# marvinx97/cloud

Hardware: AMD Instinct MI355X
Metric: images/sec ResNet-50 via run() at 1/2/4/8 MI355X; run()→first-step latency (higher is better)
Workload: dtype bf16

## Files before the change

cloud_amd/config.py:

```python
from __future__ import annotations

import os
from dataclasses import dataclass


@dataclass(frozen=True)
class Var:
    name: str
    type: type
    default: object
    doc: str
    area: str


_VARS = [
    Var("CLOUD_AMD_JOBS_DIR", str, "./jobs", "where run() stages job directories", "launcher"),
    Var("CLOUD_AMD_HOME", str, "~/.cloud_amd", "per-user state: the job-id index (jobs/<id> -> job directory) that "
        "python -m cloud_amd.jobs uses to find a job from any directory", "launcher"),
    Var("CLOUD_AMD_STAGE_COPY", bool, False, "stage code files by copying too (default: code "
        "hard-linked, every other file copied; a running job then never sees in-place edits of its sources)", "launcher"),
    Var("CLOUD_AMD_CPU_AFFINITY", bool, True, "launcher pins each GPU rank to the cores of its GPU's NUMA node "
        "(KFD io_links + sysfs cpulist), split between the ranks on that node; 0 = leave placement to the OS",
        "launcher"),
    Var("CLOUD_AMD_NUMA_ROOT", str, "/sys/devices/system/node", "sysfs NUMA-node tree read for rank CPU placement "
# ... 46 lines not shown
    Var("CLOUD_AMD_BN_APPLY_BLOCKS", int, 0, "BatchNorm apply passes (fwd y/mask, bwd dz): total workgroups of "
        "the HBM stream; 0 = the reduction kernels' tiling", "ops"),
    Var("CLOUD_AMD_BN_APPLY_ILV", bool, True, "BatchNorm apply passes: 1 = RP-row groups dealt round-robin to "
        "the workgroups (one contiguous sweep); 0 = one contiguous row chunk per workgroup", "ops"),
    Var("CLOUD_AMD_CONV_TALL", bool, True, "<= 64-channel 3x3 convolutions (fwd, stride-1 dgrad): 256 x 64 tiles "
        "with 4 x 1 waves; 0 = 128 x 64 with 2 x 2 waves", "ops"),
    Var("CLOUD_AMD_STEM_LDS", bool, True, "space-to-depth stem convolution forward on the LDS-resident patch + filter "
        "kernel (csrc/include/ca_conv_stem.h); 0 = the implicit-GEMM row-segment loader", "ops"),
    Var("CLOUD_AMD_STEM_TALL", bool, True, "space-to-depth stem convolution on the tall 256 x 64 tiles too (0.88 -> "
        "0.72 ms per call at b1024); 0 = 128 x 64 tiles (A/B runs)", "ops"),
    Var("CLOUD_AMD_STEM_BWD_RECOMPUTE", bool, True, "ResNet stem tail backward: a statistics-only max-pool "
        "backward pass, then the BN-backward apply recomputes the pooled gradient per 2x2 block (the 112x112 "
        "gradient is never written: 3.3 GB fewer per step at b1024).  With the window loads issued ahead of "
        "any branch: 0.65 + 0.90 ms against 1.09 + 0.94 for write-then-apply, +0.8 % end to end "
        "(profiles/r4_s44/); 0 = write g and run the separate apply pass", "ops"),
    Var("CLOUD_AMD_BN_GROUPS_MAX", int, 512, "BatchNorm statistics: most groups of the first-level reduction of the "
        "per-tile partial rows (1..512; ~64 rows per group)", "ops"),
    Var("CLOUD_AMD_GEMM_LIB", str, "never", "plain bf16 GEMMs (bias / accumulate only, no fused epilogue): 'never' "
        "(default: every GEMM on the in-tree kernels, the same engine on every box and rank), 'auto' (diagnostic: "
        "times the in-tree kernel against hipBLASLt once per shape and keeps the faster), 'always' "
        "(ops/raw.py PlainGemmPolicy)", "ops"),
    Var("CLOUD_AMD_GEMM_PRW", bool, True, "forward 1x1 convolutions with N = 256, K = 64 (ResNet layer-1 conv3 "
        "and shortcut): persistent resident-weight core (csrc/include/ca_gemm_prw.h); 0 = the tiled 128 core",
        "ops"),
    Var("CLOUD_AMD_GEMM_PRWN", bool, True, "forward 1x1 convolutions N = 512 / K = 128 and N = 1024 / K = 256 with "
        "BN statistics (ResNet stage-2 / stage-3 conv3): the persistent core with the weight resident in column "
        "chunks (ca_gemm_prw.h); 0 = the tiled 128 core", "ops"),
    Var("CLOUD_AMD_SMALLK_SET", str, "", "bench/smallk_gemm.py shape set ('conv3': the conv3 expansions of "
        "stages 2-4)", "bench"),
    Var("CLOUD_AMD_EPI_PF", bool, True, "GEMM epilogues that read memory or run an activation (BN-statistics "
        "forward 1x1 convs, BERT bias/GELU/GELU'/beta dense layers): 4 staged output rows in flight per trip", "ops"),
    Var("CLOUD_AMD_ATTN_FUSED_BWD", bool, True, "attention at S = 64 / 128: one workgroup per (batch, head) for "
        "the forward and a single fused backward kernel; 0 keeps the 64-query-block kernels", "ops"),
    Var("CLOUD_AMD_CONV_HALO_WGRAD", bool, True, "the weight gradient of the same 3x3 / 64-channel / width-56 "
        "convolutions on the LDS-resident kernel (ca_conv_halo.h conv3x3_halo_wgrad: 64 x 576 partial in registers, "
        "one fp32 slab per workgroup); 0 = implicit GEMM (A/B)", "ops"),
    Var("CLOUD_AMD_LN_BWD16", bool, False, "LayerNorm backward on 16-wave blocks, one row per wave, the block's "
        "partials summed by a fixed LDS tree (measured 2.8 % slower on BERT beside the weight-gradient side stream; "
        "default: 4-wave blocks walking four rows per wave)", "ops"),
    Var("CLOUD_AMD_GEMM_256X96", bool, True, "forward GEMMs whose 256 x 96 grid fills whole rounds while the 128 x "
        "128 grid leaves a partial one (BERT QKV, M = 8192, N = 2304) run on 256 x 96 tiles; 0 = off (A/B)", "ops"),
    Var("CLOUD_AMD_BN_FIN_RPG", int, 512, "BatchNorm statistics finalize: partial rows per group block (64-512)", "ops"),
    Var("CLOUD_AMD_BN_FIN_MERGED", bool, True, "BatchNorm statistics from many partial rows: group reduction and "
        "per-channel finalize in ONE launch (last block per 64 channels finalizes, agent-scope ticket); 0 = two "
        "launches (A/B runs)", "ops"),
    Var("CLOUD_AMD_CONV_HALO", int, 1, "3x3 / stride-1 / 64-channel convolutions at width 56 (ResNet-50 "
        "stage 1) forward and input gradient on the LDS-resident kernel (ca_conv_halo.h: input patch and all 9 taps "
        "in LDS, persistent grid); 0 = implicit-GEMM tiles, 2 = halo kernel without the software-pipelined "
        "fragment reads (A/B runs)", "ops"),
    Var("CLOUD_AMD_CONV_PATCH", bool, True, "3x3 / stride-1 / pad-1 convolutions with a 64-multiple gathered channel "
        "count, more than 64 output columns and W <= 28 (ResNet-50 stages 2-4), forward and input gradient, on the "
        "patch-fed core (ca_conv_patch.h: the tile's input rows go to LDS once per 64-channel chunk, not once per "
        "tap); 0 = tap-gathered implicit GEMM (A/B runs)", "ops"),
    Var("CLOUD_AMD_CONV_EPI_PF", bool, True, "implicit-GEMM forward convolutions with the BN-statistics epilogue: "
        "read 2 staged output rows from LDS before storing", "ops"),
    Var("CLOUD_AMD_SHAPE_LOG", str, None, "profiling: append one JSON line per GEMM/convolution launch (kind, M, N, "
        "K, minimum HBM bytes) to this file, for scripts/gemm_roofline.py", "ops"),
    Var("CLOUD_AMD_BN_FOLD", bool, True, "ResNet block backward: the bn3 / bn1 backward apply runs in the operand "
        "fetch of the 1x1 input-gradient GEMM that consumes it (ca_gemm_xa.h) instead of a separate pass", "ops"),
    Var("CLOUD_AMD_BN_FOLD_FWD", bool, True, "ResNet block forward: bn2's apply runs in conv3's operand fetch and "
        "bn3's (+ residual) in the next block's conv1 (ca_gemm_xa.h); the applied tensors are written once, by "
        "those GEMMs", "ops"),
    Var("CLOUD_AMD_BN_FOLD_MAX_N", int, 256, "BN fold sites kept: only GEMMs with K >= 2N and N <= this "
        "(ResNet-50 default: bn3 -> conv3 dgrad and bn3 -> next conv1 at stages 1-3, the stage-3 ones on the two-deep "
        "128 x 256 transform-A tiles, CLOUD_AMD_XA_N256=3: +0.6 / +1.0 % on two boxes, docs/performance.md round 6; "
        "4096 = every stage); the short-K sites (bn2 -> conv3, bn1 -> conv1 dgrad) measured slower than the separate "
        "pass, and stage 4 (N 512) +0.3 % below stages 1-3 only", "ops"),
    Var("CLOUD_AMD_BN_FOLD_WGRAD", bool, True, "bn3 -> conv3 fold at 64 input channels (ResNet stage 1): conv3's weight "
        "gradient runs in the same kernel as its input gradient (ca_gemm_xa.h mfma_gemm_xa_dw), so the BN-backward "
        "output dz3 is never written", "ops"),
    Var("CLOUD_AMD_BN_FOLD_DS", bool, False, "ResNet projection blocks, stages 2-4: the shortcut BN's backward apply "
        "runs in the operand fetch of the sparse strided shortcut input-gradient GEMM (ca_gemm_xa_bwd_strided); A/B",
        "ops"),
    Var("CLOUD_AMD_DS_SPARSE_DGRAD", bool, True, "ResNet projection blocks with a strided 1x1 shortcut: the "
        "shortcut's input gradient is written for its one non-empty output-parity class only, and conv1's input "
        "gradient accumulates into it reading the other pixels as zeros -- no zero-fill of 3/4 of dx and no read "
        "of those zeros", "ops"),
    Var("CLOUD_AMD_BN_FOLD_WGRAD_DS", bool, True, "stage-1 projection shortcut: its BN backward (gated by the block "
        "output's ReLU mask), the shortcut conv's input gradient and its weight gradient in one pass", "ops"),
    Var("CLOUD_AMD_BN_FOLD_WGRAD2", bool, False, "the same one-pass input + weight gradient for stage 2's conv3 "
        "(K = 512 -> N = 128, 8-wave workgroups holding the 512 x 128 dW block)", "ops"),
    Var("CLOUD_AMD_BN_FOLD_WGRAD1", bool, False, "the same one-pass input + weight gradient for stage 1's conv1 with "
        "bn1's backward apply (K = 64 -> N = 256: dz1 never written, four output chunks per tile)", "ops"),
    Var("CLOUD_AMD_XA_N256", int, 3, "transform-A GEMMs (BN folded into a 1x1 conv) with N a multiple of 256: "
        "1 = 128 x 256 tiles on 16-wave workgroups (each A tile transformed once), "
        "3 (and any other value) = 16 waves with two K tiles' operands in flight (coefficients staged in LDS; K <= 2048), "
        "0 = 128 x 128 tiles.  Only the fold sites CLOUD_AMD_BN_FOLD_MAX_N admits reach them (ResNet-50 stage 3 "
        "at the default; measured in docs/performance.md, round 6)", "ops"),
    Var("CLOUD_AMD_XA_WAVES", int, 8,"128 x 128 transform-A GEMMs (BN folded into the 1x1 convs): 8-wave "
        "workgroups (<= 128 registers, two per CU) or 4", "ops"),
    Var("CLOUD_AMD_XA_WAVES_N64", bool, True, "the 128 x 64 transform-A GEMMs (stage 1) on 8-wave workgroups too "
        "(with CLOUD_AMD_XA_WAVES=8)", "ops"),
    Var("CLOUD_AMD_XA_DW_WAVES", int, 4, "stage-1 conv3 fused input+weight gradient: 4-wave workgroups (two per "
        "CU) or 8 (one per CU); 8 selects the one-step form", "ops"),
    Var("CLOUD_AMD_XA_DW_DEPTH", int, 1, "stage-1 fused input+weight gradient (K 256 -> N 64): 0 = one-step form; "
        "1, 2, 4 = deep form (weights resident in LDS, epilogue operands ahead of the next tile's) with that many "
        "source steps in flight per workgroup (1: two workgroups per CU, 2 and 4: one)", "ops"),
    Var("CLOUD_AMD_BN_FOLD_ALL", bool, False, "fold every BN site regardless of CLOUD_AMD_BN_FOLD_MAX_N (tests, A/B)",
        "ops"),
    Var("CLOUD_AMD_MAX_STEPS_IN_FLIGHT", int, 2, "training loops (benches, Keras fit) let the host enqueue at most this "
        "many steps ahead of the GPU (runtime.step_pacer); bounds the memory in flight so the caching allocator "
        "stops requesting segments after warmup; 0 = unbounded", "runtime"),
    Var("CLOUD_AMD_RUN_AHEAD_MS", float, 25.0, "the step pacer deepens its bound (up to 4 steps) so the queued steps "
        "cover at least this much GPU time, measured on the first steps: short steps (BERT-base 8.7 ms -> 3) "
        "absorb host hiccups, long ones keep CLOUD_AMD_MAX_STEPS_IN_FLIGHT; 0 = fixed depth", "runtime"),
    Var("CLOUD_AMD_GC_FREEZE", bool, True, "training loops (benches, Keras fit) call runtime.gc_control.freeze() after "
# ... 140 lines not shown
```

cloud_amd/ops/raw.py:

```python
from __future__ import annotations

import json
import os

import torch

from . import _ext

NT, NN, TN = 0, 1, 2

_SHAPE_LOG = os.environ.get("CLOUD_AMD_SHAPE_LOG") or None


def _log(kind, M, N, K, nbytes, **kw):
    if _SHAPE_LOG is None:
        return
    with open(_SHAPE_LOG, "a") as f:
        f.write(json.dumps(dict(kind=kind, M=int(M), N=int(N), K=int(K), bytes=int(nbytes), **kw)) + "\n")


def _nb(*ts):
    if _SHAPE_LOG is None:
        return 0
    return sum(t.numel() * t.element_size() for t in ts if t is not None)
# ... 99 lines not shown
        if is_gemm_conv(w, stride, padding):
            part = torch.empty(((N * H * W + 127) // 128, 2, Cin), dtype=torch.float32, device=dy.device)
            if beta_stride > 1:
                ext.dgrad_gemm(NN, dy.data_ptr(), Cout, w.data_ptr(), Cin, dx.data_ptr(), Cin, N * H * W, Cin, Cout,
                               float(beta), 0, 0, z.data_ptr(), _ext.ptr(mask), part.data_ptr(), _st(dy.device),
                               par_s=int(beta_stride), par_h=H, par_w=W)
            else:
                ext.gemm_bf16_bnstats(NN, dy.data_ptr(), Cout, w.data_ptr(), Cin, dx.data_ptr(), Cin, N * H * W, Cin,
                                      Cout, float(beta), z.data_ptr(), _ext.ptr(mask), part.data_ptr(), _st(dy.device))
            _log("dgrad1x1_bn", N * H * W, Cin, Cout, _nb(dy, w, dx, z, mask) + (_nb(dx) if beta else 0))
        else:
            rows = ext.conv_dgrad_stat_rows(N, H, W, Cin, Cout, KH, KW, stride, stride, padding, padding,
                                            float(beta))
            part = torch.empty((rows, 2, Cin), dtype=torch.float32, device=dy.device)
            ext.conv_dgrad_bnstats(dy.data_ptr(), w.data_ptr(), dx.data_ptr(), N, H, W, Cin, Cout, KH, KW, stride,
                                   stride, padding, padding, float(beta), z.data_ptr(), _ext.ptr(mask),
                                   part.data_ptr(), _st(dy.device))
            _log("dgrad%dx%ds%d_bn" % (KH, KW, stride), N * H * W, Cin, Cout * KH * KW, _nb(dy, w, dx, z, mask),
                 launches=stride * stride)
        return dx, part
    if is_gemm_conv(w, stride, padding):
        if beta_stride > 1:
            ext.dgrad_gemm(NN, dy.data_ptr(), Cout, w.data_ptr(), Cin, dx.data_ptr(), Cin, N * H * W, Cin, Cout,
                           float(beta), 0, 0, 0, 0, 0, _st(dy.device), par_s=int(beta_stride), par_h=H, par_w=W)
        else:
            ext.gemm_bf16(NN, dy.data_ptr(), Cout, w.data_ptr(), Cin, dx.data_ptr(), Cin, N * H * W, Cin, Cout, 0,
                          float(beta), _st(dy.device))
        _log("dgrad1x1", N * H * W, Cin, Cout, _nb(dy, w, dx) + (_nb(dx) // beta_stride ** 2 if beta else 0))
        return dx
    if skip_empty:
        assert beta == 0 and stride > 1, "skip_empty: strided convolutions, beta 0"
    ext.conv_dgrad(dy.data_ptr(), w.data_ptr(), dx.data_ptr(), N, H, W, Cin, Cout, KH, KW, stride, stride, padding,
                   padding, float(beta), _st(dy.device), skip_empty=int(bool(skip_empty)))
    _log("dgrad%dx%ds%d" % (KH, KW, stride), N * H * W, Cin, Cout * KH * KW, _nb(dy, w, dx), launches=stride * stride)
    return dx


def conv_wgrad(dy, x, w_shape, stride, padding, out, beta=1.0, blocks=None):
    global _WGRAD_BLOCKS, _WGRAD_BLOCKS_SMALLM
    ext = _ext.load(required=True)
    if _WGRAD_BLOCKS is None:
        from .. import config

        _WGRAD_BLOCKS = config.get("CLOUD_AMD_WGRAD_BLOCKS")
        _WGRAD_BLOCKS_SMALLM = config.get("CLOUD_AMD_WGRAD_BLOCKS_SMALLM")
    N, H, W, Cin = x.shape
    Cout, KH, KW, _ = w_shape
    OH, OW = dy.shape[1], dy.shape[2]
    kred = N * OH * OW
    ncols = KH * KW * Cin
    target = blocks or (_WGRAD_BLOCKS_SMALLM if Cout <= 128 else _WGRAD_BLOCKS)
    splits = ext.gemm_splitk_effective(kred, wgrad_splits(Cout, ncols, kred, target_blocks=target))
    if not (KH == 1 and KW == 1):
        splits = ext.conv_wgrad_splits(N, H, W, Cin, Cout, KH, KW, stride, stride, padding, padding, splits)
    ws = torch.empty(splits * Cout * ncols, dtype=torch.float32, device=x.device)
    obf = int(out.dtype == torch.bfloat16)
    if KH == 1 and KW == 1 and stride == 1 and padding == 0:
        ext.gemm_splitk(TN, dy.data_ptr(), Cout, x.data_ptr(), Cin, out.data_ptr(), obf, float(beta), Cout, Cin,
                        kred, splits, ws.data_ptr(), _st(x.device))
    else:
        ext.conv_wgrad(dy.data_ptr(), x.data_ptr(), out.data_ptr(), obf, float(beta), N, H, W, Cin, Cout, KH, KW,
                       stride, stride, padding, padding, splits, ws.data_ptr(), _st(x.device))
    _log("wgrad%dx%ds%d" % (KH, KW, stride), Cout, ncols, kred, _nb(dy, x, out) + (2 * _nb(ws) if splits > 1 else 0),
         splits=splits)
    return out


XA_BN_RELU, XA_BN_RES_RELU, XA_BN_BWD, XA_BN_RESBN_RELU = 0, 1, 2, 3


def conv1x1_dgrad_bnbwd(dy, z, mask, coef, w, side, out=None, beta=0.0, bn=None, res=None):
    ext = _ext.load(required=True)
    N, H, W, Cout = z.shape
    Cin = w.shape[3]
    M = N * H * W
    x_shape = (N, H, W, Cin)
    assert dy.shape == z.shape and side.shape == z.shape and w.shape[1:3] == (1, 1)
    assert dy.is_contiguous() and z.is_contiguous() and side.is_contiguous() and coef.numel() == 3 * Cout
    assert mask is None or mask.shape == (M, Cout // 8)
    dx = out if out is not None else torch.empty(x_shape, dtype=torch.bfloat16, device=dy.device)
    src, rmask, zp, mp, part, part2, z2p = 0, 0, 0, 0, None, None, 0
    if res is not None:
        src_t, rm_t = res
        assert src_t.shape == dx.shape and src_t.is_contiguous()
        src, rmask = src_t.data_ptr(), _ext.ptr(rm_t)
    if bn is not None:
        zb, mb = bn[0], bn[1]
        assert zb.shape == dx.shape and zb.is_contiguous() and (mb is None or mb.shape == (M, Cin // 8))
        part = torch.empty(((M + 127) // 128, 2, Cin), dtype=torch.float32, device=dy.device)
        zp, mp = zb.data_ptr(), _ext.ptr(mb)
        if len(bn) > 2 and bn[2] is not None:
            assert res is not None, "second-BN statistics need the residual-gated (res=) form"
            part2 = torch.empty_like(part)
            z2p = bn[2].data_ptr()
    cp = coef.data_ptr()
    ext.gemm_xa(NN, XA_BN_BWD, dy.data_ptr(), z.data_ptr(), _ext.ptr(mask), cp, cp + 4 * Cout, cp + 8 * Cout, 0,
                side.data_ptr(), 0, Cout, w.data_ptr(), Cin, dx.data_ptr(), Cin, M, Cin, Cout, float(beta), src, rmask,
                zp, mp, _ext.ptr(part), z2p, _ext.ptr(part2), _st(dy.device))
    _log("dgrad1x1_xa", M, Cin, Cout, _nb(dy, z, mask, side, w, dx) + (_nb(dx) if beta else 0))
    if bn is None:
        return dx
    return (dx, part, part2) if (len(bn) > 2 and bn[2] is not None) else (dx, part)


def conv1x1_strided_dgrad_bnbwd(dy, z, mask, coef, w, side, x_shape, stride):
    ext = _ext.load(required=True)
    N, Ho, Wo, Cout = z.shape
# ... 525 lines not shown
```

csrc/bindings.cpp:

```cpp
#include <atomic>
#include <mutex>
#include <hip/hip_runtime.h>
#include <pybind11/pybind11.h>
#include <pybind11/stl.h>
#include <stdint.h>

#include <stdexcept>
#include <string>
#include <vector>

namespace py = pybind11;
typedef uint16_t bf16_t;

extern "C" {
int ca_sgd_step(float*, void*, int, float*, bf16_t*, const float*, const float*, long, int, int, hipStream_t);
int ca_adam_step(float*, void*, int, float*, float*, bf16_t*, const float*, const float*, long, int, int, hipStream_t);
int ca_rmsprop_step(float*, void*, int, float*, float*, bf16_t*, const float*, const float*, long, int, hipStream_t);
int ca_sumsq(const void*, int, long, float*, hipStream_t);
int ca_scale(void*, int, long, const float*, hipStream_t);
long ca_bn_workspace_floats(long, int);
int ca_bn_fwd(const bf16_t*, const bf16_t*, bf16_t*, long, int, const float*, const float*, float, float,
              float*, float*, float*, float*, float*, float*, int, uint8_t*, hipStream_t);
int ca_bn_apply(const bf16_t*, const bf16_t*, bf16_t*, long, int, const float*, int, hipStream_t);
int ca_bn_fwd_partials(const bf16_t*, const bf16_t*, bf16_t*, long, int, const float*, int, const float*, const float*,
                       float, float, float*, float*, float*, float*, float*, int, uint8_t*, float*, hipStream_t);
int ca_bn_bwd(const bf16_t*, const bf16_t*, const uint8_t*, const bf16_t*, long, int, const float*, const float*,
              const float*, bf16_t*, bf16_t*, float*, float*, float*, float*, int, hipStream_t);
int ca_bn_bwd_partials(const bf16_t*, const bf16_t*, const uint8_t*, const bf16_t*, long, int, const float*, int,
                       const float*, const float*, const float*, bf16_t*, bf16_t*, float*, float*, float*, float*, int,
                       hipStream_t);
int ca_gemm_bf16_bnstats(int, const bf16_t*, long, const bf16_t*, long, bf16_t*, long, int, int, int, float,
                         const bf16_t*, const uint8_t*, float*, hipStream_t);
long ca_conv_dgrad_stat_tiles(int, int, int, int, int);
long ca_conv_dgrad_stat_rows(int, int, int, int, int, int, int, int, int, int, int, float);
int ca_conv_patch_shape(int, int, int, int, int, int, int, int, int, int, int, int);
long ca_conv_stat_rows(int, int, int, int, int, int, int, int, int, int, int);
int ca_conv_wgrad_splits(int, int, int, int, int, int, int, int, int, int, int, int);
int ca_bn_fwd_partials_ex(const bf16_t*, const bf16_t*, const float*, bf16_t*, long, int, const float*, int,
                          const float*, const float*, float, float, float*, float*, float*, float*, float*, int,
                          uint8_t*, float*, hipStream_t);
int ca_gemm_xa(int, int, const bf16_t*, const bf16_t*, const uint8_t*, const float*, const float*, const float*,
               const float*, bf16_t*, uint8_t*, long, const bf16_t*, long, bf16_t*, long, int, int, int, float, const bf16_t*,
               const uint8_t*, const bf16_t*, const uint8_t*, float*, const bf16_t*, float*, hipStream_t);
int ca_gemm_xa_bwd_strided(const bf16_t*, const bf16_t*, const uint8_t*, const float*, const float*, const float*,
                           bf16_t*, long, const bf16_t*, long, bf16_t*, long, int, int, int, int, int, int, int,
                           hipStream_t);
int ca_gemm_xa_dw(const bf16_t*, const bf16_t*, const uint8_t*, const float*, const float*, const float*, long,
                  const bf16_t*, long, bf16_t*, long, int, int, int, float, const bf16_t*, const uint8_t*,
                  const bf16_t*, const uint8_t*, float*, const bf16_t*, float*, const bf16_t*, long, void*, int, float,
                  float*, int, hipStream_t);
int ca_dgrad_gemm(int, const bf16_t*, long, const bf16_t*, long, bf16_t*, long, int, int, int, float, const bf16_t*,
                  const uint8_t*, const bf16_t*, const uint8_t*, float*, hipStream_t, const bf16_t*, float*, int, int,
                  int);
int ca_conv_dgrad_bnstats(const bf16_t*, const bf16_t*, bf16_t*, int, int, int, int, int, int, int, int, int, int,
                          int, float, const bf16_t*, const uint8_t*, float*, hipStream_t);
int ca_u8_normalize(const uint8_t*, bf16_t*, long, int, const float*, const float*, hipStream_t);
int ca_stem_s2d(const bf16_t*, bf16_t*, int, int, int, int, int, int, int, hipStream_t);
int ca_softmax_xent(const void*, int, const int64_t*, int, int, float, float, float*, float*, void*, hipStream_t);
int ca_softmax_xent_batch(const void*, long, int, const int64_t*, int, int, float, float, float*, float*, void*, float*,
                          float,
                          hipStream_t);
int ca_maxpool_fwd(const bf16_t*, bf16_t*, uint8_t*, int, int, int, int, int, int, int, int, int, hipStream_t);
int ca_maxpool_bwd(const bf16_t*, const uint8_t*, bf16_t*, int, int, int, int, int, int, int, int, int, hipStream_t);
int ca_gap_fwd(const bf16_t*, void*, int, int, int, int, hipStream_t);
int ca_gap_bwd(const void*, int, bf16_t*, int, int, int, hipStream_t);
int ca_gmp_fwd(const bf16_t*, bf16_t*, float*, int, int, int, hipStream_t);
int ca_gmp_bwd(const void*, int, const bf16_t*, const bf16_t*, const float*, bf16_t*, int, int, int, hipStream_t);
int ca_gemm_bf16(int, const bf16_t*, long, const bf16_t*, long, bf16_t*, long, int, int, int, float*, float,
                 hipStream_t);
int ca_gemm_set_core(int);
int ca_gemm_set_xa_n256(int);
int ca_gemm_stat_rows(int, int, int, long, long, long);
int ca_bn_relu_maxpool_s2k3(const bf16_t*, const float*, bf16_t*, uint8_t*, int, int, int, int, int, int, hipStream_t);
int ca_maxpool_bnstats_parts(int, int, int, int);
int ca_maxpool_bwd_s2k3_bnstats(const bf16_t*, const bf16_t*, const uint8_t*, const bf16_t*, bf16_t*, float*, int, int,
                                int, int, int, int, hipStream_t);
int ca_maxpool_bwd_s2k3_bnapply(const bf16_t*, const bf16_t*, const uint8_t*, const bf16_t*, const float*, bf16_t*, int,
                                int, int, int, int, int, hipStream_t);
int ca_conv_fwd_ex(const bf16_t*, const bf16_t*, bf16_t*, int, int, int, int, int, int, int, int, int, int, int,
                   const float*, int, hipStream_t);
int ca_conv_fwd(const bf16_t*, const bf16_t*, bf16_t*, int, int, int, int, int, int, int, int, int, int, int, float*,
                hipStream_t);
int ca_conv_dgrad(const bf16_t*, const bf16_t*, bf16_t*, int, int, int, int, int, int, int, int, int, int, int, float,
                  hipStream_t, int);
int ca_conv_wgrad(const bf16_t*, const bf16_t*, void*, int, float, int, int, int, int, int, int, int, int, int, int,
                  int, int, float*, hipStream_t);
int ca_splitk_reduce(const float*, int, long, void*, int, float, hipStream_t);
int ca_grad_finalize_multi(const uint64_t*, const float*, int, hipStream_t);
int ca_cls_head_max_labels();
int ca_cls_head_fwd(const bf16_t*, long, const float*, const float*, float*, int, int, int, float, uint64_t,
// ... 151 lines not shown
                     P(bf16_t*, side),
                     P(uint8_t*, mask_out), lda, P(const bf16_t*, B), ldb, P(bf16_t*, C), ldc, M, N, K, beta,
                     P(const bf16_t*, res), P(const uint8_t*, res_mask), P(const bf16_t*, z), P(const uint8_t*, mask),
                     P(float*, stats), P(const bf16_t*, z2), P(float*, stats2), S(s)),
          "gemm_xa");
  });
  m.def("gemm_xa_bwd_strided", [](u64 src0, u64 src1, u64 mask_in, u64 c0, u64 c1, u64 c2, u64 side, long lda, u64 B,
                                  long ldb, u64 C, long ldc, int M, int N, int K, int Nb, int H, int W, int stride,
                                  u64 s) {
    check(ca_gemm_xa_bwd_strided(P(const bf16_t*, src0), P(const bf16_t*, src1), P(const uint8_t*, mask_in),
                                 P(const float*, c0), P(const float*, c1), P(const float*, c2), P(bf16_t*, side), lda,
                                 P(const bf16_t*, B), ldb, P(bf16_t*, C), ldc, M, N, K, Nb, H, W, stride, S(s)),
          "gemm_xa_bwd_strided");
  });
  m.def("gemm_xa_dw", [](u64 src0, u64 src1, u64 mask_in, u64 c0, u64 c1, u64 c2, long lda, u64 B, long ldb, u64 C,
                         long ldc, int M, int N, int K, float beta, u64 res, u64 res_mask, u64 z, u64 mask, u64 stats,
                         u64 z2, u64 stats2, u64 y, long ldy, u64 dw, int dw_bf16, float dw_beta, u64 ws, int blocks,
                         u64 s) {
    const int g = ca_gemm_xa_dw(P(const bf16_t*, src0), P(const bf16_t*, src1), P(const uint8_t*, mask_in),
                                P(const float*, c0), P(const float*, c1), P(const float*, c2), lda,
                                P(const bf16_t*, B), ldb, P(bf16_t*, C), ldc, M, N, K, beta, P(const bf16_t*, res),
                                P(const uint8_t*, res_mask), P(const bf16_t*, z), P(const uint8_t*, mask),
                                P(float*, stats), P(const bf16_t*, z2), P(float*, stats2), P(const bf16_t*, y), ldy,
                                P(void*, dw), dw_bf16, dw_beta, P(float*, ws), blocks, S(s));
    check(g < 0 ? g : 0, "gemm_xa_dw");
    return g;
  });
  m.def("bn_fwd_partials_ex", [](u64 x, u64 res, u64 res_ss, u64 y, long M, int C, u64 parts, int nparts, u64 gamma,
                                 u64 beta, float eps, float momentum, u64 rm, u64 rv, u64 sm, u64 sr, u64 ss, int relu,
                                 u64 mask, u64 gws, u64 s) {
    check(ca_bn_fwd_partials_ex(P(const bf16_t*, x), P(const bf16_t*, res), P(const float*, res_ss), P(bf16_t*, y), M,
                                C, P(const float*, parts), nparts, P(const float*, gamma), P(const float*, beta), eps,
                                momentum, P(float*, rm), P(float*, rv), P(float*, sm), P(float*, sr), P(float*, ss),
                                relu, P(uint8_t*, mask), P(float*, gws), S(s)),
          "bn_fwd_partials_ex");
  });
  m.def("conv_dgrad_stat_tiles", [](int Nb, int H, int W, int sh, int sw) {
    return ca_conv_dgrad_stat_tiles(Nb, H, W, sh, sw);
  });
  m.def("conv_dgrad_stat_rows", [](int Nb, int H, int W, int Cin, int Cout, int KH, int KW, int sh, int sw, int ph,
                                   int pw, float beta) {
    return ca_conv_dgrad_stat_rows(Nb, H, W, Cin, Cout, KH, KW, sh, sw, ph, pw, beta);
  });
  m.def("conv_stat_rows", [](int Nb, int H, int W, int Cin, int Cout, int KH, int KW, int sh, int sw, int ph,
                             int pw) { return ca_conv_stat_rows(Nb, H, W, Cin, Cout, KH, KW, sh, sw, ph, pw); });
  m.def("conv_patch_shape", [](int Nb, int H, int W, int Cin, int Cout, int KH, int KW, int sh, int sw, int ph,
                               int pw, int dgrad) {
    return ca_conv_patch_shape(Nb, H, W, Cin, Cout, KH, KW, sh, sw, ph, pw, dgrad) != 0;
  });
  m.def("conv_wgrad_splits", [](int Nb, int H, int W, int Cin, int Cout, int KH, int KW, int sh, int sw, int ph,
                                int pw, int fallback) {
    return ca_conv_wgrad_splits(Nb, H, W, Cin, Cout, KH, KW, sh, sw, ph, pw, fallback);
  });
  m.def("conv_dgrad_bnstats", [](u64 dy, u64 w, u64 dx, int Nb, int H, int W, int Cin, int Cout, int KH, int KW,
                                 int sh, int sw, int ph, int pw, float beta, u64 z, u64 mask, u64 stats, u64 s) {
    check(ca_conv_dgrad_bnstats(P(const bf16_t*, dy), P(const bf16_t*, w), P(bf16_t*, dx), Nb, H, W, Cin, Cout, KH, KW,
                                sh, sw, ph, pw, beta, P(const bf16_t*, z), P(const uint8_t*, mask), P(float*, stats),
                                S(s)),
          "conv_dgrad_bnstats");
  });
  m.def("u8_normalize", [](u64 x, u64 y, long n, std::vector<float> mean, std::vector<float> std_, u64 s) {
    if (mean.size() != std_.size() || mean.empty()) throw std::invalid_argument("u8_normalize: mean/std size");
    check(ca_u8_normalize(P(const uint8_t*, x), P(bf16_t*, y), n, (int)mean.size(), mean.data(), std_.data(), S(s)),
          "u8_normalize");
  });
  m.def("stem_s2d", [](u64 x, u64 y, int N, int H, int W, int C, int Hs, int Ws, int pad, u64 s) {
    check(ca_stem_s2d(P(const bf16_t*, x), P(bf16_t*, y), N, H, W, C, Hs, Ws, pad, S(s)), "stem_s2d");
  });
  m.def("softmax_xent", [](u64 z, int zbf, u64 labels, int B, int C, float gscale, float ls, u64 loss, u64 correct,
                           u64 dz, u64 s) {
    check(ca_softmax_xent(P(const void*, z), zbf, P(const int64_t*, labels), B, C, gscale, ls, P(float*, loss),
                          P(float*, correct), P(void*, dz), S(s)), "softmax_xent");
  });
  m.def("softmax_xent_batch", [](u64 z, long ldz, int bf, u64 labels, int B, int C, float gs, float ls, u64 mean, u64 correct,
                                 u64 dz, u64 acc, float acc_w, u64 s) {
    check(ca_softmax_xent_batch(P(const void*, z), ldz, bf, P(const int64_t*, labels), B, C, gs, ls, P(float*, mean),
                                P(float*, correct), P(void*, dz), P(float*, acc), acc_w, S(s)), "softmax_xent_batch");
  });
  m.def("maxpool_fwd", [](u64 x, u64 y, u64 idx, int N, int H, int W, int C, int OH, int OW, int k, int st, int p,
                          u64 s) {
    check(ca_maxpool_fwd(P(const bf16_t*, x), P(bf16_t*, y), P(uint8_t*, idx), N, H, W, C, OH, OW, k, st, p, S(s)),
          "maxpool_fwd");
  });
  m.def("maxpool_bwd", [](u64 dy, u64 idx, u64 dx, int N, int H, int W, int C, int OH, int OW, int k, int st, int p,
                          u64 s) {
    check(ca_maxpool_bwd(P(const bf16_t*, dy), P(const uint8_t*, idx), P(bf16_t*, dx), N, H, W, C, OH, OW, k, st, p,
                         S(s)), "maxpool_bwd");
  });
  m.def("gap_fwd", [](u64 x, u64 y, int ybf, int N, int HW, int C, u64 s) {
    check(ca_gap_fwd(P(const bf16_t*, x), P(void*, y), ybf, N, HW, C, S(s)), "gap_fwd");
  });
  m.def("gemm_bf16", [](int layout, u64 A, long lda, u64 B, long ldb, u64 C, long ldc, int M, int N, int K,
                        u64 stats, float beta, u64 s) {
    check(ca_gemm_bf16(layout, P(const bf16_t*, A), lda, P(const bf16_t*, B), ldb, P(bf16_t*, C), ldc, M, N, K,
                       P(float*, stats), beta, S(s)), "gemm_bf16");
  });
  m.def("conv_fwd", [](u64 x, u64 w, u64 y, int Nb, int H, int W, int Cin, int Cout, int KH, int KW, int sh, int sw,
                       int ph, int pw, u64 stats, u64 s) {
    check(ca_conv_fwd(P(const bf16_t*, x), P(const bf16_t*, w), P(bf16_t*, y), Nb, H, W, Cin, Cout, KH, KW, sh, sw, ph,
                      pw, P(float*, stats), S(s)), "conv_fwd");
  });
  m.def("bn_relu_maxpool_s2k3", [](u64 z, u64 ss, u64 y, u64 idx, int N, int H, int W, int C, int OH, int OW,
                                   u64 s) {
    check(ca_bn_relu_maxpool_s2k3(P(const bf16_t*, z), P(const float*, ss), P(bf16_t*, y), P(uint8_t*, idx), N, H, W,
                                  C, OH, OW, S(s)), "bn_relu_maxpool_s2k3");
  });
// ... 147 lines not shown
```

csrc/kernels/conv.hip:

```cpp
#include <stdlib.h>
#include <string.h>

#include "ca_conv_halo.h"
#include "ca_conv_patch.h"
#include "ca_conv_stem.h"
#include "ca_mfma_core.h"

namespace {
using namespace ca;

struct Pix {
  int n, y, x;
};
__device__ __forceinline__ Pix decode(uint32_t m, const FastDiv& dw, const FastDiv& dh) {
  const uint32_t t = fdiv(m, dw);
  const uint32_t x = m - t * dw.d;
  const uint32_t n = fdiv(t, dh);
  return Pix{(int)n, (int)(t - n * dh.d), (int)x};
}

__device__ __forceinline__ void tap_split(int k, int k0, int C, const FastDiv& dc, bool tile_in_tap, int& tap,
                                          int& c) {
  tap = (int)fdiv((uint32_t)(tile_in_tap ? k0 : k), dc);
  c = k - tap * C;
}

template <int R, int CPT, int NT>
struct ConvFwdA {
  static constexpr bool KC = true;
  const CoreParams& P;
  const bf16_t* nbase[CPT];
  int iy0[CPT], ix0[CPT], col[CPT];
  __device__ ConvFwdA(const CoreParams& p, bool, int r0, int tid) : P(p) {
#pragma unroll
    for (int i = 0; i < CPT; ++i) {
      int row, c;
      chunk_coords<R, true>(tid + i * NT, row, c);
      const int m = r0 + row;
      col[i] = c;
      if (m < P.M) {
        const Pix o = decode((uint32_t)m, P.div_ow, P.div_oh);
        nbase[i] = P.A + (long)o.n * P.H * P.W * P.Cin;
        iy0[i] = o.y * P.sh - P.ph;
        ix0[i] = o.x * P.sw - P.pw;
      } else {
        nbase[i] = P.A;
        iy0[i] = -(1 << 29);
        ix0[i] = 0;
      }
    }
  }
  __device__ __forceinline__ s8v load(int i, int k0) const {
    const int k = k0 + col[i];
    if (k >= P.K) return zero8();
    int tap, ci;
    tap_split(k, k0, P.Cin, P.div_cin, P.cin_tile, tap, ci);
    const int kh = (int)fdiv((uint32_t)tap, P.div_kw), kw = tap - kh * P.KW;
// ... 651 lines not shown
  return on;
}

bool use_glds() {
  static const bool glds = [] {
    const char* e = getenv("CLOUD_AMD_GEMM_CORE");
    return !(e && e[0] == 'r');
  }();
  return glds;
}

bool tapmask_loaders() {
  static const bool on = env_switch("CLOUD_AMD_TAPMASK", true);
  return on;
}

template <int PROWS, bool DGRAD, template <int, int, int> class LB, int EPI, int EPF = 1>
__global__ void __launch_bounds__(256) __attribute__((amdgpu_waves_per_eu(4))) conv_patch_kernel(CoreParams P) {
  conv_patch_gemm<PROWS, DGRAD, LB, EPI, EPF>(P);
}

bool conv_patch_on() {
  static const bool on = env_switch("CLOUD_AMD_CONV_PATCH", true);
  return on;
}

bool patch_shape(int Nb, int H, int W, int C, int NC, int KH, int KW, int sh, int sw, int ph, int pw) {
  return conv_patch_on() && KH == 3 && KW == 3 && sh == 1 && sw == 1 && ph == 1 && pw == 1 && C % BK == 0 &&
         NC > 64 && W <= PATCH_MAXW && use_glds() && tapmask_loaders() && (long)Nb * H * W * C * 2 < (long)BUF_CAP;
}

template <int PROWS, bool DGRAD, template <int, int, int> class LB, int EPI>
int launch_patch_rows(const CoreParams& p, int tiles, hipStream_t s) {
  if constexpr (EPI == EPI_BF16_ST) {
    if (conv_epi_pf()) {
      conv_patch_kernel<PROWS, DGRAD, LB, EPI, 2><<<dim3(tiles, 1, 1), 256, 0, s>>>(p);
      CA_LAUNCH_CHECK();
      return 0;
    }
  }
  conv_patch_kernel<PROWS, DGRAD, LB, EPI><<<dim3(tiles, 1, 1), 256, 0, s>>>(p);
  CA_LAUNCH_CHECK();
  return 0;
}

template <bool DGRAD, template <int, int, int> class LB, int EPI>
int launch_patch(const CoreParams& p0, hipStream_t s) {
  CoreParams p = p0;
  p.split_xcd = split_xcd_enabled();
  const int tiles = ((p.M + 127) / 128) * ((p.N + 127) / 128);
  if (patch_rows(p.W) <= 160) return launch_patch_rows<160, DGRAD, LB, EPI>(p, tiles, s);
  return launch_patch_rows<192, DGRAD, LB, EPI>(p, tiles, s);
}

template <int BM, int BN, template <int, int, int> class LA, template <int, int, int> class LB, int EPI>
__global__ void __launch_bounds__(256) conv_gemm_kernel(CoreParams P) {
  mfma_gemm_body<BM, BN, 2, 2, LA, LB, EPI, 2>(P);
}

template <int BM, int BN, template <int, int, int> class LA, template <int, int, int> class LB,
          template <int, int, int> class GA, template <int, int, int> class GB, int EPI>
int launch(const CoreParams& p0, int splits, hipStream_t s) {
  CoreParams p = p0;
  p.split_xcd = split_xcd_enabled();
  const int tiles = ((p.M + BM - 1) / BM) * ((p.N + BN - 1) / BN);
  if constexpr (EPI == EPI_BF16_ST) {
    if (use_glds() && conv_epi_pf()) {
      conv_glds_kernel<BM, BN, GA, GB, EPI, 2><<<dim3(tiles, 1, splits), 256, 0, s>>>(p);
      CA_LAUNCH_CHECK();
      return 0;
    }
  }
  if (use_glds()) {
    conv_glds_kernel<BM, BN, GA, GB, EPI><<<dim3(tiles, 1, splits), 256, 0, s>>>(p);
    CA_LAUNCH_CHECK();
    return 0;
  }
  conv_gemm_kernel<BM, BN, LA, LB, EPI><<<dim3(tiles, 1, splits), 256, 0, s>>>(p);
  CA_LAUNCH_CHECK();
  return 0;
}

template <template <int, int, int> class LA, template <int, int, int> class LB,
          template <int, int, int> class GA, template <int, int, int> class GB, int EPI>
int launch_n64(const CoreParams& p0, hipStream_t s) {
  if (!(tall_tiles() && use_glds())) return launch<128, 64, LA, LB, GA, GB, EPI>(p0, 1, s);
  CoreParams p = p0;
  p.split_xcd = split_xcd_enabled();
  const int tiles = (p.M + 255) / 256;
  if constexpr (EPI == EPI_BF16_ST) {
    if (conv_epi_pf()) {
      conv_glds_w_kernel<256, 64, 4, 1, GA, GB, EPI, 2><<<dim3(tiles, 1, 1), 256, 0, s>>>(p);
      CA_LAUNCH_CHECK();
      return 0;
    }
  }
  conv_glds_w_kernel<256, 64, 4, 1, GA, GB, EPI><<<dim3(tiles, 1, 1), 256, 0, s>>>(p);
  CA_LAUNCH_CHECK();
  return 0;
}

template <int STATS, bool PIPE>
__global__ void __launch_bounds__(HALO_NT) conv3x3_halo_kernel(HaloParams P) {
  conv3x3_halo<STATS, PIPE>(P);
}

// ... 247 lines not shown
        q.div_hq = make_fastdiv(q.Hq);
        q.div_wq = make_fastdiv(q.Wq);
        q.div_nw = make_fastdiv(q.dg_nw > 0 ? q.dg_nw : 1);
        q.M = Nb * q.Hq * q.Wq;
        q.K = q.dg_nh * q.dg_nw * Cout;
        q.k_per_split = q.K;
        if (bnz) {
          q.stats = stats + stat_row * 2 * Cin;
          stat_row += (q.M + 127) / 128;
        }
        int rc = bnz ? launch_dgrad_s<EPI_BF16_BN>(q, Cin, s) : launch_dgrad_s<EPI_BF16>(q, Cin, s);
        if (rc) return rc;
      }
    return 0;
  }
  return bnz ? launch_dgrad<EPI_BF16_BN>(p, Cin, s) : launch_dgrad<EPI_BF16>(p, Cin, s);
}

extern "C" {

int ca_conv_dgrad(const bf16_t* dy, const bf16_t* w, bf16_t* dx, int Nb, int H, int W, int Cin, int Cout, int KH,
                  int KW, int sh, int sw, int ph, int pw, float beta, hipStream_t s, int skip_empty) {
  if (skip_empty && (beta != 0.f || (sh == 1 && sw == 1))) return -1;
  return conv_dgrad_impl(dy, w, dx, Nb, H, W, Cin, Cout, KH, KW, sh, sw, ph, pw, beta, nullptr, nullptr, nullptr, s,
                         skip_empty);
}

int ca_conv_dgrad_bnstats(const bf16_t* dy, const bf16_t* w, bf16_t* dx, int Nb, int H, int W, int Cin, int Cout,
                          int KH, int KW, int sh, int sw, int ph, int pw, float beta, const bf16_t* bnz,
                          const uint8_t* bnmask, float* stats, hipStream_t s) {
  if (!bnz || !stats) return -1;
  return conv_dgrad_impl(dy, w, dx, Nb, H, W, Cin, Cout, KH, KW, sh, sw, ph, pw, beta, bnz, bnmask, stats, s);
}

int ca_conv_wgrad(const bf16_t* dy, const bf16_t* x, void* dw, int dw_bf16, float beta, int Nb, int H, int W,
                  int Cin, int Cout, int KH, int KW, int sh, int sw, int ph, int pw, int splits, float* ws,
                  hipStream_t s) {
  if (halo_shape(H, W, Cin, Cout, KH, KW, sh, sw, ph, pw) && halo_wgrad_on() && splits == halo_grid(Nb, H)) {
    HaloWgParams hp{x, dy, ws, Nb, H, W};
    conv3x3_halo_wgrad_kernel<<<splits, HWG_NT, 0, s>>>(hp);
    CA_LAUNCH_CHECK();
    return ca_splitk_reduce(ws, splits, (long)Cout * KH * KW * Cin, dw, dw_bf16, beta, s);
  }
  CoreParams p = conv_params(Nb, H, W, Cin, Cout, KH, KW, sh, sw, ph, pw);
  if (!geom_ok(Cin, Cout, (long)Nb * H * W)) return -1;
  p.A = dy; p.lda = Cout; p.B = x;
  p.M = Cout; p.N = KH * KW * Cin; p.K = Nb * p.OH * p.OW;
  int kps = (p.K / splits + BK - 1) / BK * BK;
  if (kps < BK) kps = BK;
  splits = (p.K + kps - 1) / kps;
  p.k_per_split = kps;
  p.C = ws; p.ldc = p.N; p.split_stride = (long)p.M * p.N;
  int rc;
  if (tapmask_loaders() && (long)p.OH * p.OW >= 2 * BK) {
    if (Cout <= 64)
      rc = (p.N <= 64) ? launch<64, 64, DenseNC, ConvWgradB, GDenseNC, GConvWgradBI, EPI_F32_PARTIAL>(p, splits, s)
                       : launch<64, 128, DenseNC, ConvWgradB, GDenseNC, GConvWgradBI, EPI_F32_PARTIAL>(p, splits, s);
    else
      rc = (p.N <= 64) ? launch<128, 64, DenseNC, ConvWgradB, GDenseNC, GConvWgradBI, EPI_F32_PARTIAL>(p, splits, s)
                       : launch<128, 128, DenseNC, ConvWgradB, GDenseNC, GConvWgradBI, EPI_F32_PARTIAL>(p, splits, s);
    if (rc) return rc;
    return ca_splitk_reduce(ws, splits, (long)p.M * p.N, dw, dw_bf16, beta, s);
  }
  if (tapmask_loaders()) {
    if (Cout <= 64)
      rc = (p.N <= 64) ? launch<64, 64, DenseNC, ConvWgradB, GDenseNC, GConvWgradBT, EPI_F32_PARTIAL>(p, splits, s)
                       : launch<64, 128, DenseNC, ConvWgradB, GDenseNC, GConvWgradBT, EPI_F32_PARTIAL>(p, splits, s);
    else
      rc = (p.N <= 64) ? launch<128, 64, DenseNC, ConvWgradB, GDenseNC, GConvWgradBT, EPI_F32_PARTIAL>(p, splits, s)
                       : launch<128, 128, DenseNC, ConvWgradB, GDenseNC, GConvWgradBT, EPI_F32_PARTIAL>(p, splits, s);
    if (rc) return rc;
    return ca_splitk_reduce(ws, splits, (long)p.M * p.N, dw, dw_bf16, beta, s);
  }
  if (Cout <= 64)
    rc = (p.N <= 64) ? launch<64, 64, DenseNC, ConvWgradB, GDenseNC, GConvWgradB, EPI_F32_PARTIAL>(p, splits, s)
                     : launch<64, 128, DenseNC, ConvWgradB, GDenseNC, GConvWgradB, EPI_F32_PARTIAL>(p, splits, s);
  else
    rc = (p.N <= 64) ? launch<128, 64, DenseNC, ConvWgradB, GDenseNC, GConvWgradB, EPI_F32_PARTIAL>(p, splits, s)
                     : launch<128, 128, DenseNC, ConvWgradB, GDenseNC, GConvWgradB, EPI_F32_PARTIAL>(p, splits, s);
  if (rc) return rc;
  return ca_splitk_reduce(ws, splits, (long)p.M * p.N, dw, dw_bf16, beta, s);
}

int ca_conv_wgrad_splits(int Nb, int H, int W, int Cin, int Cout, int KH, int KW, int sh, int sw, int ph, int pw,
                         int fallback) {
  if (halo_shape(H, W, Cin, Cout, KH, KW, sh, sw, ph, pw) && halo_wgrad_on()) return halo_grid(Nb, H);
  return fallback;
}

int ca_conv_patch_shape(int Nb, int H, int W, int Cin, int Cout, int KH, int KW, int sh, int sw, int ph, int pw,
                        int dgrad) {
  return dgrad ? patch_shape(Nb, H, W, Cout, Cin, KH, KW, sh, sw, ph, pw)
               : patch_shape(Nb, H, W, Cin, Cout, KH, KW, sh, sw, ph, pw);
}

int ca_conv_out_hw(int H, int KH, int sh, int ph) { return (H + 2 * ph - KH) / sh + 1; }

}
```

Baseline: 16390.

## Add patch-fed split-K kernel for 3x3 weight gradients in ResNet stages 2-4

Adds a new weight-gradient kernel for 3x3 stride-1 convolutions with Cin a multiple of 64 and at least 128 output channels. Each block loads the input rows once into LDS and the three taps of a filter row read shifted views of that copy, rather than gathering each tap separately. It also adds a split-count heuristic that targets three resident blocks per CU with a minimum K per split. The aim is less global/LDS traffic in the wgrad GEMMs, at the cost of a fixed 128-row M tile and a new boundary-masking path.

```diff
diff --git a/cloud_amd/config.py b/cloud_amd/config.py
--- a/cloud_amd/config.py
+++ b/cloud_amd/config.py
@@ -122,6 +122,10 @@
         "count, more than 64 output columns and W <= 28 (ResNet-50 stages 2-4), forward and input gradient, on the "
         "patch-fed core (ca_conv_patch.h: the tile's input rows go to LDS once per 64-channel chunk, not once per "
         "tap); 0 = tap-gathered implicit GEMM (A/B runs)", "ops"),
+    Var("CLOUD_AMD_CONV_PATCH_WGRAD", bool, True, "3x3 / stride-1 / pad-1 weight gradients with Cin a multiple of 64, "
+        "at least 128 output channels and W <= 28 (ResNet-50 stages 2-4) on the patch-fed split-K core "
+        "(ca_conv_patch_wgrad.h: the three taps of a filter row read one LDS copy of the input rows); "
+        "0 = tap-gathered implicit GEMM (A/B runs)", "ops"),
     Var("CLOUD_AMD_CONV_EPI_PF", bool, True, "implicit-GEMM forward convolutions with the BN-statistics epilogue: "
         "read 2 staged output rows from LDS before storing", "ops"),
     Var("CLOUD_AMD_SHAPE_LOG", str, None, "profiling: append one JSON line per GEMM/convolution launch (kind, M, N, "
diff --git a/cloud_amd/ops/raw.py b/cloud_amd/ops/raw.py
--- a/cloud_amd/ops/raw.py
+++ b/cloud_amd/ops/raw.py
@@ -175,7 +175,8 @@
     target = blocks or (_WGRAD_BLOCKS_SMALLM if Cout <= 128 else _WGRAD_BLOCKS)
     splits = ext.gemm_splitk_effective(kred, wgrad_splits(Cout, ncols, kred, target_blocks=target))
     if not (KH == 1 and KW == 1):
-        splits = ext.conv_wgrad_splits(N, H, W, Cin, Cout, KH, KW, stride, stride, padding, padding, splits)
+        splits = ext.conv_wgrad_splits(N, H, W, Cin, Cout, KH, KW, stride, stride, padding, padding, splits,
+                                       int(target), 64 if blocks else 512)
     ws = torch.empty(splits * Cout * ncols, dtype=torch.float32, device=x.device)
     obf = int(out.dtype == torch.bfloat16)
     if KH == 1 and KW == 1 and stride == 1 and padding == 0:
diff --git a/csrc/bindings.cpp b/csrc/bindings.cpp
--- a/csrc/bindings.cpp
+++ b/csrc/bindings.cpp
@@ -36,6 +36,8 @@
 int ca_conv_patch_shape(int, int, int, int, int, int, int, int, int, int, int, int);
 long ca_conv_stat_rows(int, int, int, int, int, int, int, int, int, int, int);
 int ca_conv_wgrad_splits(int, int, int, int, int, int, int, int, int, int, int, int);
+int ca_conv_wgrad_splits_ex(int, int, int, int, int, int, int, int, int, int, int, int, int, int);
+int ca_conv_wgrad_patch_shape(int, int, int, int, int, int, int, int, int, int, int);
 int ca_bn_fwd_partials_ex(const bf16_t*, const bf16_t*, const float*, bf16_t*, long, int, const float*, int,
                           const float*, const float*, float, float, float*, float*, float*, float*, float*, int,
                           uint8_t*, float*, hipStream_t);
@@ -293,6 +295,14 @@
                                 int pw, int fallback) {
     return ca_conv_wgrad_splits(Nb, H, W, Cin, Cout, KH, KW, sh, sw, ph, pw, fallback);
   });
+  m.def("conv_wgrad_splits", [](int Nb, int H, int W, int Cin, int Cout, int KH, int KW, int sh, int sw, int ph,
+                                int pw, int fallback, int blocks, int min_k) {
+    return ca_conv_wgrad_splits_ex(Nb, H, W, Cin, Cout, KH, KW, sh, sw, ph, pw, fallback, blocks, min_k);
+  });
+  m.def("conv_wgrad_patch_shape", [](int Nb, int H, int W, int Cin, int Cout, int KH, int KW, int sh, int sw, int ph,
+                                     int pw) {
+    return ca_conv_wgrad_patch_shape(Nb, H, W, Cin, Cout, KH, KW, sh, sw, ph, pw) != 0;
+  });
   m.def("conv_dgrad_bnstats", [](u64 dy, u64 w, u64 dx, int Nb, int H, int W, int Cin, int Cout, int KH, int KW,
                                  int sh, int sw, int ph, int pw, float beta, u64 z, u64 mask, u64 stats, u64 s) {
     check(ca_conv_dgrad_bnstats(P(const bf16_t*, dy), P(const bf16_t*, w), P(bf16_t*, dx), Nb, H, W, Cin, Cout, KH, KW,
diff --git a/csrc/include/ca_conv_patch_wgrad.h b/csrc/include/ca_conv_patch_wgrad.h
--- /dev/null
+++ b/csrc/include/ca_conv_patch_wgrad.h
@@ -0,0 +1,166 @@
+#pragma once
+#include "ca_conv_patch.h"
+
+namespace ca {
+
+constexpr int PWG_BM = 128;
+constexpr int PWG_ROWS = 72;
+constexpr int PWG_ZROW = 66;
+
+__device__ __forceinline__ void conv_patch_wgrad_gemm(const CoreParams& P) {
+  constexpr int BM = PWG_BM, NT = 256, WN = 2, FM = 4, FN = 6;
+  constexpr int A_ELEMS = BK * BM, P_ELEMS = PWG_ROWS * BK;
+  constexpr int CPA = A_ELEMS / 8 / NT;
+  using LA = GDenseNC<BM, CPA, NT>;
+  __shared__ __attribute__((aligned(16))) short smem[A_ELEMS + P_ELEMS];
+
+  const int tid = threadIdx.x, lane = tid & 63, wave = tid >> 6;
+  const int wm = wave / WN, wn = wave % WN;
+  const int W = P.W, H = P.H, C = P.Cin;
+  const int nchunk = C / BK;
+  const BlkPos bp = blk_pos(P);
+  const int t3 = bp.tile / nchunk;
+  const int c0 = (bp.tile - t3 * nchunk) * BK;
+  const int tm = t3 / 3, kh = t3 - tm * 3;
+  const int m0 = tm * BM;
+  const int kbeg = bp.split * P.k_per_split;
+  int kend = kbeg + P.k_per_split;
+  if (kend > P.K) kend = P.K;
+  const int nk = (kend - kbeg + BK - 1) / BK;
+
+  const LA la(P, true, m0, tid);
+  const auto ra = loader_rsrc(la);
+  const uint32_t x_span = buf_span((long)P.K * C * 2);
+  const auto rx = __builtin_amdgcn_make_buffer_rsrc(const_cast<bf16_t*>(P.B), (short)0, (int)x_span, 0x00020000);
+
+  const int row_t = tid >> 3;
+  const int pcol = ((tid & 7) ^ nc_swz<64>(row_t)) << 3;
+  int pixr = kbeg + (kh - 1) * W - 1 + row_t;
+  uint32_t offr = ((uint32_t)pixr * (uint32_t)C + (uint32_t)(c0 + pcol)) * 2u;
+  const uint32_t tile_step = (uint32_t)(BK * C * 2), grp_step = (uint32_t)(32 * C * 2);
+  short* const Pd = smem + A_ELEMS;
+  auto issue = [&](int t) {
+    const int k0 = kbeg + t * BK;
+#pragma unroll
+    for (int i = 0; i < CPA; ++i)
+      __builtin_amdgcn_raw_ptr_buffer_load_lds(ra, (lds_void*)(smem + (i * NT + wave * 64) * 8), 16, la.off(i, k0), 0, 0, 0);
+#pragma unroll
+    for (int i = 0; i < 2; ++i) {
+      const bool ok = (unsigned)(pixr + 32 * i) < (unsigned)P.K;
+      const uint32_t o = ok ? offr + (uint32_t)i * grp_step : x_span;
+      __builtin_amdgcn_raw_ptr_buffer_load_lds(rx, (lds_void*)(Pd + (i * NT + wave * 64) * 8), 16, o, 0, 0, 0);
+    }
+    if (wave == 0) {
+      const bool ok = (unsigned)(pixr + 64) < (unsigned)P.K && row_t < PWG_ZROW - 64;
+      const uint32_t o = ok ? offr + 2u * grp_step : x_span;
+      __builtin_amdgcn_raw_ptr_buffer_load_lds(rx, (lds_void*)(Pd + 2 * NT * 8), 16, o, 0, 0, 0);
+    }
+    pixr += BK;
+    offr += tile_step;
+  };
+
+  const int g = lane >> 4, q = (lane & 15) >> 2, p = lane & 3;
+  const int kl = 8 * g + q;
+  int bcol[2][3], brow[2][3], bzero[2][3];
+#pragma unroll
+  for (int hf = 0; hf < 2; ++hf)
+#pragma unroll
+    for (int kw = 0; kw < 3; ++kw) {
+      const int pr = kl + 4 * hf + kw;
+      bcol[hf][kw] = (((wn * 4 + (p >> 1)) ^ nc_swz<64>(pr)) << 3) + 4 * (p & 1);
+      brow[hf][kw] = pr * BK;
+      bzero[hf][kw] = (PWG_ZROW + (pr & 1)) * BK;
+    }
+
+  int py[4], px[4];
+#pragma unroll
+  for (int r = 0; r < 4; ++r) {
+    const uint32_t k = (uint32_t)(kbeg + kl + 4 * (r & 1) + 32 * (r >> 1));
+    const uint32_t t = fdiv(k, P.div_w);
+    px[r] = (int)(k - t * (uint32_t)W);
+    py[r] = (int)(t - fdiv(t, P.div_h) * (uint32_t)H);
+  }
+  const int dya = (int)fdiv((uint32_t)BK, P.div_w);
+  const int dxa = BK - dya * W;
+  const int dym = dya - (int)fdiv((uint32_t)dya, P.div_h) * H;
+  int kcur = kbeg + kl;
+
+  f4v acc[FM][FN];
+#pragma unroll
+  for (int i = 0; i < FM; ++i)
+#pragma unroll
+    for (int j = 0; j < FN; ++j) acc[i][j] = f4v{0.f, 0.f, 0.f, 0.f};
+
+  auto compute = [&]() {
+    const short* const As = smem;
+    const short* const Ps = smem + A_ELEMS;
+#pragma unroll
+    for (int hi = 0; hi < 2; ++hi) {
+      int ba[2][3];
+#pragma unroll
+      for (int hf = 0; hf < 2; ++hf) {
+        const int r = 2 * hi + hf;
+        const bool rok = (kcur + 4 * hf + 32 * hi < P.K) & ((unsigned)(py[r] + kh - 1) < (unsigned)H);
+        const bool ok[3] = {rok && px[r] >= 1, rok, rok && px[r] + 1 < W};
+#pragma unroll
+        for (int kw = 0; kw < 3; ++kw)
+          ba[hf][kw] = (ok[kw] ? brow[hf][kw] + 32 * hi * BK : bzero[hf][kw]) + bcol[hf][kw];
+      }
+      bf16x8 af[FM];
+#pragma unroll
+      for (int i = 0; i < FM; ++i) af[i] = read_frag_sw<BM, false>(As, wm * 64 + i * 16, hi * 32, lane);
+#pragma unroll
+      for (int kw = 0; kw < 3; ++kw) {
+        bf16x8 bfr[2];
+#pragma unroll
+        for (int h = 0; h < 2; ++h) {
+          const s4v lo = __builtin_amdgcn_ds_read_tr16_b64_v4i16((lds_s4v*)(Ps + (ba[0][kw] ^ (h << 4))));
+          const s4v up = __builtin_amdgcn_ds_read_tr16_b64_v4i16((lds_s4v*)(Ps + (ba[1][kw] ^ (h << 4))));
+          const s8v v = {lo[0], lo[1], lo[2], lo[3], up[0], up[1], up[2], up[3]};
+          bfr[h] = __builtin_bit_cast(bf16x8, v);
+        }
+#pragma unroll
+        for (int i = 0; i < FM; ++i)
+#pragma unroll
+          for (int h = 0; h < 2; ++h)
+            acc[i][kw * 2 + h] = __builtin_amdgcn_mfma_f32_16x16x32_bf16(bfr[h], af[i], acc[i][kw * 2 + h], 0, 0, 0);
+      }
+    }
+    kcur += BK;
+#pragma unroll
+    for (int r = 0; r < 4; ++r) {
+      int x = px[r] + dxa, y = py[r] + dym;
+      if (x >= W) {
+        x -= W;
+        y += 1;
+      }
+      if (y >= H) y -= H;
+      px[r] = x;
+      py[r] = y;
+    }
+  };
+
+  for (int t = 0; t < nk; ++t) {
+    issue(t);
+    asm volatile("s_waitcnt vmcnt(0)" ::: "memory");
+    __syncthreads();
+    compute();
+    __syncthreads();
+  }
+
+  float* const Cp = reinterpret_cast<float*>(P.C) + (long)bp.split * P.split_stride;
+#pragma unroll
+  for (int i = 0; i < FM; ++i) {
+    const int gm = m0 + wm * 64 + i * 16 + (lane & 15);
+    if (gm >= P.M) continue;
+#pragma unroll
+    for (int kw = 0; kw < 3; ++kw)
+#pragma unroll
+      for (int h = 0; h < 2; ++h) {
+        const int gn = (kh * 3 + kw) * C + c0 + wn * 32 + h * 16 + 4 * g;
+        *reinterpret_cast<f4v*>(Cp + (long)gm * P.ldc + gn) = acc[i][kw * 2 + h];
+      }
+  }
+}
+
+}
diff --git a/csrc/kernels/conv.hip b/csrc/kernels/conv.hip
--- a/csrc/kernels/conv.hip
+++ b/csrc/kernels/conv.hip
@@ -3,6 +3,7 @@
 
 #include "ca_conv_halo.h"
 #include "ca_conv_patch.h"
+#include "ca_conv_patch_wgrad.h"
 #include "ca_conv_stem.h"
 #include "ca_mfma_core.h"
 
@@ -760,6 +761,26 @@
   if (patch_rows(p.W) <= 160) return launch_patch_rows<160, DGRAD, LB, EPI>(p, tiles, s);
   return launch_patch_rows<192, DGRAD, LB, EPI>(p, tiles, s);
 }
+
+__global__ void __launch_bounds__(256) __attribute__((amdgpu_waves_per_eu(3))) conv_patch_wgrad_kernel(CoreParams P) {
+  conv_patch_wgrad_gemm(P);
+}
+
+bool conv_patch_wgrad_on() {
+  static const bool on = env_switch("CLOUD_AMD_CONV_PATCH_WGRAD", true);
+  return on;
+}
+
+bool patch_wgrad_shape(int Nb, int H, int W, int Cin, int Cout, int KH, int KW, int sh, int sw, int ph, int pw) {
+  const long pix = (long)Nb * H * W;
+  return conv_patch_wgrad_on() && KH == 3 && KW == 3 && sh == 1 && sw == 1 && ph == 1 && pw == 1 && Cin % BK == 0 &&
+         Cout >= PWG_BM && Cout % 8 == 0 && W <= PATCH_MAXW && use_glds() && tapmask_loaders() && pix > 0 &&
+         pix < (1L << 31) && pix * (Cin > Cout ? Cin : Cout) * 2 < (long)BUF_CAP;
+}
+
+int patch_wgrad_tiles(int Cin, int Cout) { return ((Cout + PWG_BM - 1) / PWG_BM) * 3 * (Cin / BK); }
+
+constexpr int PWG_RESIDENT = 3;
 
 template <int BM, int BN, template <int, int, int> class LA, template <int, int, int> class LB, int EPI>
 __global__ void __launch_bounds__(256) conv_gemm_kernel(CoreParams P) {
@@ -1113,6 +1134,12 @@
   p.k_per_split = kps;
   p.C = ws; p.ldc = p.N; p.split_stride = (long)p.M * p.N;
   int rc;
+  if (patch_wgrad_shape(Nb, H, W, Cin, Cout, KH, KW, sh, sw, ph, pw)) {
+    p.split_xcd = split_xcd_enabled();
+    conv_patch_wgrad_kernel<<<dim3(patch_wgrad_tiles(Cin, Cout), 1, splits), 256, 0, s>>>(p);
+    CA_LAUNCH_CHECK();
+    return ca_splitk_reduce(ws, splits, (long)p.M * p.N, dw, dw_bf16, beta, s);
+  }
   if (tapmask_loaders() && (long)p.OH * p.OW >= 2 * BK) {
     if (Cout <= 64)
       rc = (p.N <= 64) ? launch<64, 64, DenseNC, ConvWgradB, GDenseNC, GConvWgradBI, EPI_F32_PARTIAL>(p, splits, s)
@@ -1143,10 +1170,30 @@
   return ca_splitk_reduce(ws, splits, (long)p.M * p.N, dw, dw_bf16, beta, s);
 }
 
+int ca_conv_wgrad_splits_ex(int Nb, int H, int W, int Cin, int Cout, int KH, int KW, int sh, int sw, int ph, int pw,
+                            int fallback, int blocks, int min_k) {
+  if (halo_shape(H, W, Cin, Cout, KH, KW, sh, sw, ph, pw) && halo_wgrad_on()) return halo_grid(Nb, H);
+  if (patch_wgrad_shape(Nb, H, W, Cin, Cout, KH, KW, sh, sw, ph, pw)) {
+    const int K = Nb * H * W, tiles = patch_wgrad_tiles(Cin, Cout);
+    const int target = blocks > 0 ? blocks : PWG_RESIDENT * conv_cus();
+    if (min_k <= 0) min_k = 512;
+    const int kmax = min_k <= BK ? (K + BK - 1) / BK : (K / min_k > 1 ? K / min_k : 1);
+    int splits = (target + tiles - 1) / tiles;
+    if (splits > kmax) splits = kmax;
+    const int kps = (K / splits + BK - 1) / BK * BK;
+    return (K + kps - 1) / kps;
+  }
+  return fallback;
+}
+
 int ca_conv_wgrad_splits(int Nb, int H, int W, int Cin, int Cout, int KH, int KW, int sh, int sw, int ph, int pw,
                          int fallback) {
-  if (halo_shape(H, W, Cin, Cout, KH, KW, sh, sw, ph, pw) && halo_wgrad_on()) return halo_grid(Nb, H);
-  return fallback;
+  return ca_conv_wgrad_splits_ex(Nb, H, W, Cin, Cout, KH, KW, sh, sw, ph, pw, fallback, 0, 0);
+}
+
+int ca_conv_wgrad_patch_shape(int Nb, int H, int W, int Cin, int Cout, int KH, int KW, int sh, int sw, int ph,
+                              int pw) {
+  return patch_wgrad_shape(Nb, H, W, Cin, Cout, KH, KW, sh, sw, ph, pw);
 }
 
 int ca_conv_patch_shape(int Nb, int H, int W, int Cin, int Cout, int KH, int KW, int sh, int sw, int ph, int pw,
```

New measurement: 16460, median of 6. About the same (+0.4%).
